# jerry102102102/RL_brain_trainer

Hardware: AMD Instinct MI355X
Metric: env-steps/sec (whole node), Stage-5 Approach->Finisher PPO loops (rollout + update); value = the Approach loop, finisher.value = the Finisher loop (higher is better)
Workload: dtype f32

## Files before the change

### rl_brain_trainer_amd/csrc/kp1_mlp.hip

```cpp
#include <hip/hip_runtime.h>
#include <hip/hip_ext.h>

#include <cmath>
#include <cstddef>
#include <cstdlib>
#include <cstring>
#include <vector>

#include "../../include/kp1_ppo.h"
#include "kp1_device.hpp"
#include "kp1_host.hpp"

using kp1::fail;
using namespace kp1;

typedef float f32x16 __attribute__((ext_vector_type(16)));
typedef float f32x4 __attribute__((ext_vector_type(4)));

namespace {

constexpr int ACT = KP1_MLP_ACT, HEADS = 8;
constexpr float LOG_SQRT_2PI = 0.9189385332046727f;

enum { EPI_BIAS_TANH = 0, EPI_DTANH = 1 };
// ... 1177 lines not shown
  if (g.reps > 1) {
    if (g.N != 128) return fail(KP1_ERR_UNSUPPORTED, "population gemm_nt is instantiated for N = 128");
    if (g.K == 64) return launch_nt_inst<128, EPI, 64, true>(g, stream);
    if (g.K == 128) return launch_nt_inst<128, EPI, 128, true>(g, stream);
    return fail(KP1_ERR_UNSUPPORTED, "population gemm_nt is instantiated for K in {64, 128}");
  }
  const int row_tiles = (g.M + 63) / 64;
  const bool wide = (g.N % 256 == 0) && row_tiles * 2 >= 200;
  if (g.K == 64) return wide ? launch_nt_inst<256, EPI, 64>(g, stream) : launch_nt_inst<128, EPI, 64>(g, stream);
  if (g.K == 128) return wide ? launch_nt_inst<256, EPI, 128>(g, stream) : launch_nt_inst<128, EPI, 128>(g, stream);
  if (g.K == 256) return wide ? launch_nt_inst<256, EPI, 256>(g, stream) : launch_nt_inst<128, EPI, 256>(g, stream);
  return fail(KP1_ERR_UNSUPPORTED, "gemm_nt is instantiated for K in {64, 128, 256}");
}

int launch_tn(kp1_mlp* m, GemmTN t, int n_o_tiles, int slab_cols, float* slab, int* n_chunks_out, hipStream_t stream);

int launch_fused(const FusedArgs& fa_in, hipStream_t stream) {
  FusedArgs fa = fa_in;
  static const int stagger_us = [] { const char* e = std::getenv("KP1_FU_STAGGER_US"); return e ? std::atoi(e) : 11; }();
  static const int n_cus = [] {
    int dev = 0, n = 0;
    if (hipGetDevice(&dev) != hipSuccess || hipDeviceGetAttribute(&n, hipDeviceAttributeMultiprocessorCount, dev) != hipSuccess) n = 256;
    return n;
  }();
  const dim3 grid((fa.n + FU_BM - 1) / FU_BM, 1, 2);
  fa.n_cus = n_cus;
  fa.stagger_ticks = (int)(grid.x * grid.z) > n_cus ? stagger_us * 100 : 0;
  const size_t bytes = sizeof(float) * FU_LDS_FLOATS;
  if (fa.sp_h1 != nullptr) {
    if (fa.inp == 64) {
      HIP_TRY(hipFuncSetAttribute((const void*)mlp_tile_kernel<true, 2, 0, true>, hipFuncAttributeMaxDynamicSharedMemorySize, (int)bytes));
      KP1_LAUNCH((mlp_tile_kernel<true, 2, 0, true>), grid, dim3(FU_NTH), bytes, stream, fa);
    } else {
      HIP_TRY(hipFuncSetAttribute((const void*)mlp_tile_kernel<true, 4, 0, true>, hipFuncAttributeMaxDynamicSharedMemorySize, (int)bytes));
      KP1_LAUNCH((mlp_tile_kernel<true, 4, 0, true>), grid, dim3(FU_NTH), bytes, stream, fa);
    }
    return KP1_OK;
  }
  if (fa.inp == 64) {
    HIP_TRY(hipFuncSetAttribute((const void*)mlp_tile_kernel<true, 2>, hipFuncAttributeMaxDynamicSharedMemorySize, (int)bytes));
    KP1_LAUNCH((mlp_tile_kernel<true, 2>), grid, dim3(FU_NTH), bytes, stream, fa);
  } else {
    HIP_TRY(hipFuncSetAttribute((const void*)mlp_tile_kernel<true, 4>, hipFuncAttributeMaxDynamicSharedMemorySize, (int)bytes));
    KP1_LAUNCH((mlp_tile_kernel<true, 4>), grid, dim3(FU_NTH), bytes, stream, fa);
  }
  return KP1_OK;
}

int launch_fused_infer_env(const FusedArgs& fa, int env_mode, hipStream_t stream) {
  const size_t bytes = sizeof(float) * FU_LDS_FLOATS;
  const dim3 grid((fa.n + FU_BM - 1) / FU_BM, 1, fa.value ? 2 : 1);
  if (env_mode == KP1_MODE_DOCK) {
    HIP_TRY(hipFuncSetAttribute((const void*)mlp_tile_kernel<false, 2, 2>, hipFuncAttributeMaxDynamicSharedMemorySize, (int)bytes));
    hipLaunchKernelGGL((mlp_tile_kernel<false, 2, 2>), grid, dim3(FU_NTH), bytes, stream, fa);
  } else {
    HIP_TRY(hipFuncSetAttribute((const void*)mlp_tile_kernel<false, 2, 1>, hipFuncAttributeMaxDynamicSharedMemorySize, (int)bytes));
    hipLaunchKernelGGL((mlp_tile_kernel<false, 2, 1>), grid, dim3(FU_NTH), bytes, stream, fa);
  }
  return KP1_OK;
}

int launch_fused_infer(const FusedArgs& fa, hipStream_t stream) {
  const size_t bytes = sizeof(float) * FU_LDS_FLOATS;
  const bool want_pi = fa.mean || fa.action || fa.clipped || fa.log_prob;
  if (!want_pi && !fa.value) return KP1_OK;
  FusedArgs f = fa;
  const bool both = want_pi && fa.value;
  if (!both) f.net_base = want_pi ? 0 : 1;
  const dim3 grid((fa.n + FU_BM - 1) / FU_BM, 1, both ? 2 : 1);
  if (fa.inp == 64) {
    HIP_TRY(hipFuncSetAttribute((const void*)mlp_tile_kernel<false, 2>, hipFuncAttributeMaxDynamicSharedMemorySize, (int)bytes));
    hipLaunchKernelGGL((mlp_tile_kernel<false, 2>), grid, dim3(FU_NTH), bytes, stream, f);
  } else {
    HIP_TRY(hipFuncSetAttribute((const void*)mlp_tile_kernel<false, 4>, hipFuncAttributeMaxDynamicSharedMemorySize, (int)bytes));
    hipLaunchKernelGGL((mlp_tile_kernel<false, 4>), grid, dim3(FU_NTH), bytes, stream, f);
  }
  return KP1_OK;
}

int launch_tn_frag(const TnFragArgs& t, hipStream_t stream) {
  if (t.n_chunks2 > 64 || t.n_chunks1 > 64) return fail(KP1_ERR_INVALID, "too many batch chunks for the partial-gradient slabs");
  const size_t bytes = sizeof(float) * TN_SPLIT_LDS_FLOATS;
  HIP_TRY(hipFuncSetAttribute((const void*)gemm_tn_split_kernel, hipFuncAttributeMaxDynamicSharedMemorySize, (int)bytes));
  KP1_LAUNCH(gemm_tn_split_kernel, dim3(32 * t.n_chunks2 + 16 * t.n_chunks1), dim3(256), bytes, stream, t);
  return KP1_OK;
}

int launch_forward_layers(kp1_mlp* m, const float* obs, int obs_stride, const int64_t* idx, int n, hipStream_t stream) {
  const int Hp = m->Hp, IN = m->L.IN, INP = m->L.INP;
  const int64_t act_stride = (int64_t)m->max_batch * Hp;
  GemmNT g{};
  g.reps = m->K;
  g.r_A = idx ? 0u : (unsigned)(n * obs_stride); g.r_gather = (unsigned)n;
  g.r_W = (unsigned)(2 * Hp * INP); g.r_bias = (unsigned)(2 * Hp); g.r_C = (unsigned)(2 * act_stride);
  g.A = obs; g.lda = obs_stride; g.strideA = 0; g.gather = idx;
  g.W = m->k.w1p; g.strideW = (int64_t)Hp * INP;
  g.bias = m->k.b1; g.strideBias = Hp;
  g.C = m->h1; g.ldc = Hp; g.strideC = act_stride;
  g.aux = nullptr; g.strideAux = 0; g.colsum = nullptr; g.strideColsum = 0;
  g.M = n; g.N = Hp; g.K = INP; g.Kreal = obs_stride >= INP ? INP : IN;
  int rc = launch_nt<EPI_BIAS_TANH>(g, stream);
  if (rc != KP1_OK) return rc;
  g.A = m->h1; g.lda = Hp; g.strideA = act_stride; g.gather = nullptr;
  g.r_A = (unsigned)(2 * act_stride); g.r_W = (unsigned)(2 * Hp * Hp);
  g.W = m->k.w2; g.strideW = (int64_t)Hp * Hp;
  g.bias = m->k.b2;
  g.C = m->h2;
  g.K = Hp; g.Kreal = Hp;
  rc = launch_nt<EPI_BIAS_TANH>(g, stream);
  if (rc != KP1_OK) return rc;
  HIP_TRY(kp1::launch_status());
  return KP1_OK;
}

}

namespace {
int launch_tn(kp1_mlp* m, GemmTN t, int n_o_tiles, int slab_cols, float* slab, int* n_chunks_out, hipStream_t stream) {
  const int Hp = m->Hp;
  const int n_chunks = (t.B + t.chunk - 1) / t.chunk;
  if (n_chunks > 64) return fail(KP1_ERR_INVALID, "too many batch chunks for the partial-gradient slab");
  t.slab = slab;
  t.slab_ld = slab_cols;
  t.slab_net_stride = (int64_t)Hp * slab_cols;
  t.slab_chunk_stride = 2 * t.slab_net_stride;
  const dim3 grid(n_chunks, n_o_tiles * t.n_i_tiles, 2 * m->K);
  if (m->K > 1) {
    t.reps = m->K;
    t.r_D = (unsigned)(2 * (int64_t)m->max_batch * Hp);
    t.r_X = t.gatherX ? 0u : t.r_D;
    t.r_gather = (unsigned)t.B;
    t.r_slab = (unsigned)(64 * t.slab_chunk_stride);
    if (t.gatherX) {
      HIP_TRY(hipFuncSetAttribute((const void*)gemm_tn_kernel<true, true>, hipFuncAttributeMaxDynamicSharedMemorySize, (int)TN_LDS_BYTES));
      hipLaunchKernelGGL((gemm_tn_kernel<true, true>), grid, dim3(256), TN_LDS_BYTES, stream, t);
    } else {
      HIP_TRY(hipFuncSetAttribute((const void*)gemm_tn_kernel<false, true>, hipFuncAttributeMaxDynamicSharedMemorySize, (int)TN_LDS_BYTES));
      hipLaunchKernelGGL((gemm_tn_kernel<false, true>), grid, dim3(256), TN_LDS_BYTES, stream, t);
    }
  } else if (t.gatherX) {
    HIP_TRY(hipFuncSetAttribute((const void*)gemm_tn_kernel<true>, hipFuncAttributeMaxDynamicSharedMemorySize, (int)TN_LDS_BYTES));
    hipLaunchKernelGGL(gemm_tn_kernel<true>, grid, dim3(256), TN_LDS_BYTES, stream, t);
  } else {
    HIP_TRY(hipFuncSetAttribute((const void*)gemm_tn_kernel<false>, hipFuncAttributeMaxDynamicSharedMemorySize, (int)TN_LDS_BYTES));
    hipLaunchKernelGGL(gemm_tn_kernel<false>, grid, dim3(256), TN_LDS_BYTES, stream, t);
  }
  if (n_chunks_out) *n_chunks_out = n_chunks;
  return KP1_OK;
}
}

extern "C" {

int64_t kp1_mlp_num_params(int32_t hidden) { return hidden > 0 ? make_layout(hidden).total : 0; }
int64_t kp1_mlp_num_params_ex(int32_t hidden, int32_t obs_dim) { return hidden > 0 && obs_dim > 0 && obs_dim <= 128 ? make_layout(hidden, obs_dim).total : 0; }

int kp1_mlp_create(int32_t device, int32_t hidden, int32_t max_batch, kp1_mlp** out) { return kp1_mlp_create_ex(device, hidden, KP1_MLP_IN, max_batch, out); }

namespace {
int mlp_create(int32_t device, int32_t hidden, int32_t obs_dim, int32_t max_batch, int32_t replicas, kp1_mlp** out);
}

int kp1_mlp_create_ex(int32_t device, int32_t hidden, int32_t obs_dim, int32_t max_batch, kp1_mlp** out) {
  return mlp_create(device, hidden, obs_dim, max_batch, 1, out);
}

int kp1_mlp_create_population(int32_t device, int32_t hidden, int32_t obs_dim, int32_t max_batch, int32_t replicas, kp1_mlp** out) {
// ... 271 lines not shown
  }
  const int hpart_stride = 10 * Hp + 32;
  if (fused) {
    FusedArgs fa{};
    fa.obs = obs; fa.obs_stride = obs_stride; fa.Kreal = obs_stride >= INP ? INP : IN; fa.inp = INP; fa.idx = idx; fa.n = n;
    fa.k = m->k;
    fa.actions = actions; fa.old_logp = old_log_prob; fa.adv = advantages; fa.ret = returns;
    fa.adv_partials = m->partials; fa.n_adv_partials = N_PARTIALS; fa.adv_stats = adv_stats_dev; fa.adv_mean = adv_mean; fa.adv_inv_std = adv_inv_std;
    fa.adv_mode = adv_mode;
    fa.clip_range = clip_range; fa.vf_coef = vf_coef; fa.inv_count = inv_count;
    fa.h1 = m->h1; fa.dz2 = m->dz2; fa.dz1 = m->dz1; fa.act_stride = act_stride; fa.xf = m->xf;
    fa.bslab = m->bslab; fa.hpart = m->hpart; fa.hpart_stride = hpart_stride;
    if (m->bf16x3) {
      fa.sp_h1 = m->sp_h1; fa.sp_dz2 = m->sp_dz2; fa.sp_dz1 = m->sp_dz1; fa.sp_xf = m->sp_xf;
      fa.sp_plane = (int64_t)2 * m->max_batch * Hp; fa.sp_plane_x = (int64_t)m->max_batch * INP;
    }
    {
      ProfScope ps(m, KP1_MLP_PROFILE_TILE, stream);
      rc = launch_fused(fa, stream);
    }
    if (rc != KP1_OK) return rc;
  } else {
    rc = launch_forward_layers(m, obs, obs_stride, idx, n, stream);
    if (rc != KP1_OK) return rc;
    HeadArgs a{};
    a.h2 = m->h2; a.strideH = act_stride; a.Hp = Hp; a.n = n; a.H = H;
    a.w3 = m->k.w3; a.b3 = m->k.b3; a.log_std = m->k.log_std;
    a.idx = idx; a.actions = actions; a.old_logp = old_log_prob; a.adv = advantages; a.ret = returns;
    a.adv_partials = m->partials; a.n_adv_partials = N_PARTIALS; a.adv_stats = adv_stats_dev; a.adv_mean = adv_mean; a.adv_inv_std = adv_inv_std;
    a.adv_mode = adv_mode;
    a.clip_range = clip_range; a.ent_coef = ent_coef; a.vf_coef = vf_coef; a.inv_count = inv_count;
    a.dz2 = m->dz2;
    a.hpart = m->hpart; a.hpart_stride = hpart_stride;
    a.r_act = (unsigned)(2 * act_stride); a.r_hpart = (unsigned)hpart_rep; a.r_partials = (unsigned)PARTIALS_STRIDE;
    a.hparams = pop && m->hparams_on ? m->hparams_dev : nullptr;
    {
      const dim3 hgrid((n + HEAD_ROWS - 1) / HEAD_ROWS, m->K);
      const size_t hbytes = sizeof(float) * (HEADS * Hp + HEAD_ROWS * 8 + 84 + 2 * HEAD_ROWS * (Hp + 4));
      if (pop) {
        HIP_TRY(hipFuncSetAttribute((const void*)head_train_kernel<128, true>, hipFuncAttributeMaxDynamicSharedMemorySize, (int)hbytes));
        hipLaunchKernelGGL((head_train_kernel<128, true>), hgrid, dim3(256), hbytes, stream, a);
      } else if (Hp == 256) {
        HIP_TRY(hipFuncSetAttribute((const void*)head_train_kernel<256>, hipFuncAttributeMaxDynamicSharedMemorySize, (int)hbytes));
        hipLaunchKernelGGL(head_train_kernel<256>, hgrid, dim3(256), hbytes, stream, a);
      } else {
        HIP_TRY(hipFuncSetAttribute((const void*)head_train_kernel<128>, hipFuncAttributeMaxDynamicSharedMemorySize, (int)hbytes));
        hipLaunchKernelGGL(head_train_kernel<128>, hgrid, dim3(256), hbytes, stream, a);
      }
    }
    GemmNT g{};
    g.A = m->dz2; g.lda = Hp; g.strideA = act_stride; g.gather = nullptr;
    g.W = m->k.w2t; g.strideW = (int64_t)Hp * Hp;
    g.bias = nullptr; g.strideBias = 0;
    g.C = m->dz1; g.ldc = Hp; g.strideC = act_stride;
    g.aux = m->h1; g.strideAux = act_stride;
    g.colsum = m->bslab; g.strideColsum = Hp;
    g.M = n; g.N = Hp; g.K = Hp; g.Kreal = Hp;
    g.reps = m->K;
    g.r_A = g.r_C = g.r_aux = (unsigned)(2 * act_stride); g.r_W = (unsigned)(2 * Hp * Hp);
    g.r_colsum = (unsigned)((m->max_batch / 32) * 2 * Hp);
    rc = launch_nt<EPI_DTANH>(g, stream);
    if (rc != KP1_OK) return rc;
  }

  int s2_n = 0, s1_n = 0;
  if (fused) {
    TnFragArgs t{};
    t.inp = INP;
    t.dz2 = m->dz2; t.h1 = m->h1; t.dz1 = m->dz1; t.act_stride = act_stride; t.xf = m->xf;
    t.slab2 = m->slab; t.s2_net = (int64_t)Hp * Hp; t.s2_chunk = 2 * t.s2_net;
    t.slab1 = m->slab1; t.s1_net = (int64_t)Hp * INP; t.s1_chunk = 2 * t.s1_net;
    t.groups = (n + FU_BM - 1) / FU_BM * (FU_BM / 8);
    auto up8 = [](int v) { return (v + 7) / 8 * 8; };
    t.cg2 = up8((t.groups + TN_SPLIT2 - 1) / TN_SPLIT2);
    t.cg1 = up8((t.groups + TN_SPLIT1 - 1) / TN_SPLIT1);
    t.n_chunks2 = (t.groups + t.cg2 - 1) / t.cg2;
    t.n_chunks1 = (t.groups + t.cg1 - 1) / t.cg1;
    if (m->bf16x3) {
      TnBf16Args b{};
      b.dz2 = m->sp_dz2; b.h1 = m->sp_h1; b.dz1 = m->sp_dz1; b.plane = (int64_t)2 * m->max_batch * Hp; b.net = (int64_t)m->max_batch * Hp;
      b.xf = m->sp_xf; b.plane_x = (int64_t)m->max_batch * INP; b.inp = INP;
      b.slab2 = t.slab2; b.s2_net = t.s2_net; b.s2_chunk = t.s2_chunk; b.slab1 = t.slab1; b.s1_net = t.s1_net; b.s1_chunk = t.s1_chunk;
      b.frags = t.groups / 2; b.cf2 = t.cg2 / 2; b.cf1 = t.cg1 / 2; b.n_chunks2 = t.n_chunks2; b.n_chunks1 = t.n_chunks1;
      const size_t bytes = sizeof(float) * TN_SPLIT_LDS_FLOATS;
      HIP_TRY(hipFuncSetAttribute((const void*)gemm_tn_bf16x3_kernel, hipFuncAttributeMaxDynamicSharedMemorySize, (int)bytes));
      ProfScope ps(m, KP1_MLP_PROFILE_WGRAD, stream);
      KP1_LAUNCH(gemm_tn_bf16x3_kernel, dim3(32 * b.n_chunks2 + 16 * b.n_chunks1), dim3(256), bytes, stream, b);
    } else {
      ProfScope ps(m, KP1_MLP_PROFILE_WGRAD, stream);
      rc = launch_tn_frag(t, stream);
    }
    if (rc != KP1_OK) return rc;
    s2_n = t.n_chunks2;
    s1_n = t.n_chunks1;
  } else {
    GemmTN t{};
    t.B = n;
    t.chunk = tn_chunk_rows(n, (Hp / 128) * (Hp / 128) * 2);
    t.D = m->dz2; t.ldd = Hp; t.strideD = act_stride;
    t.X = m->h1; t.ldx = Hp; t.strideX = act_stride; t.gatherX = nullptr;
    t.Nload = Hp; t.n_i_tiles = Hp / 128;
    rc = launch_tn(m, t, Hp / 128, Hp, m->slab, &s2_n, stream);
    if (rc != KP1_OK) return rc;
    t.D = m->dz1;
    t.X = obs; t.ldx = obs_stride; t.strideX = 0; t.gatherX = idx;
    t.Nload = obs_stride >= INP ? INP : IN; t.n_i_tiles = 1;
    t.chunk = tn_chunk_rows(n, (Hp / 128) * 2);
    rc = launch_tn(m, t, Hp / 128, INP, m->slab1, &s1_n, stream);
    if (rc != KP1_OK) return rc;
  }
  FinalizeArgs f{};
  f.L = L;
  f.slab2 = m->slab; f.s2_ld = Hp; f.s2_net = (int64_t)Hp * Hp; f.s2_chunk = 2 * f.s2_net; f.s2_n = s2_n;
  f.slab1 = m->slab1; f.s1_ld = INP; f.s1_net = (int64_t)Hp * INP; f.s1_chunk = 2 * f.s1_net; f.s1_n = s1_n;
  f.bslab = m->bslab; f.b_net = Hp; f.b_tile = 2 * Hp; f.b_n = fused ? (n + FU_BM - 1) / FU_BM * (FU_BM / 32) : nt_row_tiles(n, Hp);
  f.hpart = m->hpart; f.h_stride = 10 * Hp + 32; f.h_n = (n + HEAD_ROWS - 1) / HEAD_ROWS;
  f.ent_coef = ent_coef; f.inv_count = inv_count; f.log_std = m->k.log_std;
  f.grad = grad_out; f.stats = stats_out; f.sumsq = m->partials + 2 * N_PARTIALS;
  f.step_counter = m->step_dev;
  f.r_slab2 = (unsigned)(64 * f.s2_chunk); f.r_slab1 = (unsigned)(64 * f.s1_chunk); f.r_bslab = (unsigned)((m->max_batch / 32) * 2 * Hp);
  f.r_hpart = (unsigned)hpart_rep; f.r_sumsq = (unsigned)PARTIALS_STRIDE;
  f.hparams = pop && m->hparams_on ? m->hparams_dev : nullptr;
  const int n_main = (int)((finalize_vec_items(L) + 255) / 256);
  m->n_finalize_blocks = n_main + (int)((finalize_wide_count(L) + 3 + 31) / 32);
  if (m->n_finalize_blocks > 2048) return fail(KP1_ERR_INVALID, "parameter vector too large for the sum-of-squares partial buffer");
  {
    ProfScope ps(m, KP1_MLP_PROFILE_FINALIZE, stream);
    if (pop)
      KP1_LAUNCH(grad_finalize_kernel<true>, dim3(m->n_finalize_blocks, m->K), dim3(256), 0, stream, f, n_main);
    else
      KP1_LAUNCH(grad_finalize_kernel<false>, dim3(m->n_finalize_blocks), dim3(256), 0, stream, f, n_main);
  }
  HIP_TRY(kp1::launch_status());
  return KP1_OK;
}

int kp1_mlp_profile_read(kp1_mlp* m, float* out_us, int32_t* out_launches) {
  if (!m || !out_us || !out_launches) return fail(KP1_ERR_INVALID, "NULL argument to kp1_mlp_profile_read");
  int rc = mlp_check_device(m);
  if (rc != KP1_OK) return rc;
  for (int k = 0; k < KP1_MLP_PROFILE_SLOTS; ++k) {
    double total_ms = 0.0;
    for (int i = 0; i < m->prof_used[k]; ++i) {
      HIP_TRY(hipEventSynchronize(m->prof[k][i].b));
      float ms = 0.f;
      HIP_TRY(hipEventElapsedTime(&ms, m->prof[k][i].a, m->prof[k][i].b));
      total_ms += ms;
    }
    out_launches[k] = m->prof_used[k];
    out_us[k] = m->prof_used[k] > 0 ? (float)(total_ms * 1e3 / m->prof_used[k]) : 0.f;
    m->prof_used[k] = 0;
  }
  return KP1_OK;
}

int kp1_mlp_time_kernels(kp1_mlp* m, const float* obs, int32_t obs_stride, int32_t n, int32_t iters, float* out_ms, double* out_flops,
                         void* stream_) {
  if (!m || !obs || !out_ms || !out_flops || iters <= 0) return fail(KP1_ERR_INVALID, "bad argument to kp1_mlp_time_kernels");
  if (m->K > 1) return fail(KP1_ERR_UNSUPPORTED, "kp1_mlp_time_kernels is not available on population handles");
  if (n <= 0 || n > m->max_batch) return fail(KP1_ERR_INVALID, "n exceeds the workspace max_batch");
  int rc = mlp_check_device(m);
  if (rc != KP1_OK) return rc;
  hipStream_t stream = (hipStream_t)stream_;
  const int Hp = m->Hp, IN = m->L.IN, INP = m->L.INP;
  const int64_t act_stride = (int64_t)m->max_batch * Hp;
  hipEvent_t e0, e1;
  HIP_TRY(hipEventCreate(&e0));
// ... 78 lines not shown
  }
  (void)hipEventDestroy(e0);
  (void)hipEventDestroy(e1);
  return KP1_OK;
}

__global__ void __launch_bounds__(FU_NTH, 2) placement_probe_kernel(unsigned int* __restrict__ where, unsigned int* __restrict__ arrived, unsigned int total) {
  extern __shared__ float lds[];
  if (threadIdx.x == 0) {
    const unsigned int hw = __builtin_amdgcn_s_getreg((31 << 11) | 4);
    const unsigned int xcc = __builtin_amdgcn_s_getreg((3 << 11) | 20);
    const unsigned int linear = blockIdx.x + gridDim.x * blockIdx.z;
    where[linear] = (xcc << 16) | (((hw >> 13) & 7u) << 8) | (((hw >> 12) & 1u) << 4) | ((hw >> 8) & 15u);
    lds[0] = 0.f;
    __hip_atomic_fetch_add(arrived, 1u, __ATOMIC_RELAXED, __HIP_MEMORY_SCOPE_AGENT);
    const unsigned long long t0 = wall_clock64();
    while (__hip_atomic_load(arrived, __ATOMIC_RELAXED, __HIP_MEMORY_SCOPE_AGENT) < total && wall_clock64() - t0 < 200000ull) __builtin_amdgcn_s_sleep(8);
  }
  __syncthreads();
}

int kp1_mlp_placement_check(int32_t device, int32_t n_rows, int32_t* out, void* stream_) {
  if (!out || n_rows <= 0) return fail(KP1_ERR_INVALID, "bad argument to kp1_mlp_placement_check");
  HIP_TRY(hipSetDevice(device));
  hipStream_t stream = (hipStream_t)stream_;
  int n_cus = 0;
  HIP_TRY(hipDeviceGetAttribute(&n_cus, hipDeviceAttributeMultiprocessorCount, device));
  const dim3 grid((n_rows + FU_BM - 1) / FU_BM, 1, 2);
  const unsigned int total = grid.x * grid.z;
  if ((int)total > 2 * n_cus) return fail(KP1_ERR_UNSUPPORTED, "placement probe: the grid must be resident at once");
  unsigned int* dev = nullptr;
  HIP_TRY(hipMalloc(&dev, sizeof(unsigned int) * (total + 1)));
  HIP_TRY(hipMemsetAsync(dev, 0, sizeof(unsigned int) * (total + 1), stream));
  const size_t bytes = sizeof(float) * FU_LDS_FLOATS;
  HIP_TRY(hipFuncSetAttribute((const void*)placement_probe_kernel, hipFuncAttributeMaxDynamicSharedMemorySize, (int)bytes));
  hipLaunchKernelGGL(placement_probe_kernel, grid, dim3(FU_NTH), bytes, stream, dev, dev + total, total);
  std::vector<unsigned int> host(total + 1);
  hipError_t e = hipMemcpyAsync(host.data(), dev, sizeof(unsigned int) * (total + 1), hipMemcpyDeviceToHost, stream);
  if (e == hipSuccess) e = hipStreamSynchronize(stream);
  (void)hipFree(dev);
  HIP_TRY(e);
  int pairs = 0, same = 0, rr = 0;
  std::vector<unsigned int> seen;
  for (unsigned int k = 0; k < total; ++k) {
    if ((host[k] >> 16) == (host[k & 7u] >> 16)) ++rr;
    if (k + (unsigned)n_cus < total) {
      ++pairs;
      if (host[k] == host[k + n_cus]) ++same;
    }
    bool fresh = true;
    for (unsigned int v : seen) fresh = fresh && v != host[k];
    if (fresh) seen.push_back(host[k]);
  }
  int xcds = 0;
  for (unsigned int a = 0; a < 8 && a < total; ++a) {
    bool fresh = true;
    for (unsigned int b = 0; b < a; ++b) fresh = fresh && (host[a] >> 16) != (host[b] >> 16);
    xcds += fresh ? 1 : 0;
  }
  out[0] = (int)total; out[1] = pairs; out[2] = same; out[3] = rr; out[4] = n_cus; out[5] = (int)seen.size(); out[6] = (int)host[total]; out[7] = xcds;
  return KP1_OK;
}

#ifdef KP1_CLK_TRACE
int kp1_debug_clk_trace(unsigned long long* out) {
  HIP_TRY(hipDeviceSynchronize());
  HIP_TRY(hipMemcpyFromSymbol(out, HIP_SYMBOL(kp1_clk_buf), sizeof(unsigned long long) * 2 * 1024 * 4));
  return KP1_OK;
}
#endif

#ifdef KP1_NT_TRACE
int kp1_debug_nt_trace(unsigned long long* out, int clear) {
  HIP_TRY(hipDeviceSynchronize());
  if (out) HIP_TRY(hipMemcpyFromSymbol(out, HIP_SYMBOL(kp1_nt_trace_buf), sizeof(unsigned long long) * KP1_TRACE_SLOTS * KP1_TRACE_WGS));
  if (clear) {
    std::vector<unsigned long long> z(KP1_TRACE_SLOTS * KP1_TRACE_WGS, 0ull);
    HIP_TRY(hipMemcpyToSymbol(HIP_SYMBOL(kp1_nt_trace_buf), z.data(), sizeof(unsigned long long) * z.size()));
  }
  return KP1_OK;
}
#endif

int kp1_mlp_adam_step(kp1_mlp* m, float* params, float* grad, float* exp_avg, float* exp_avg_sq, float lr, float eps, float max_grad_norm,
                      int32_t step, int32_t zero_grad, void* stream_) {
  if (!m || !params || !grad || !exp_avg || !exp_avg_sq) return fail(KP1_ERR_INVALID, "bad argument to kp1_mlp_adam_step");
  int rc = mlp_check_device(m);
  if (rc != KP1_OK) return rc;
  hipStream_t stream = (hipStream_t)stream_;
  const int64_t n = m->L.total;
  const bool fused_norm = (zero_grad & 2) && m->n_finalize_blocks > 0;
  const double* norm_partials = fused_norm ? m->partials + 2 * N_PARTIALS : m->partials + N_PARTIALS;
  const int n_norm_partials = fused_norm ? m->n_finalize_blocks : N_PARTIALS;
  ProfScope ps(m, KP1_MLP_PROFILE_ADAM, stream);
  const bool pop = m->K > 1;
  if (!fused_norm) {
    if (pop)
      hipLaunchKernelGGL(sumsq_partials_kernel<true>, dim3(N_PARTIALS, m->K), dim3(256), 0, stream, grad, n, m->partials + N_PARTIALS, (unsigned)PARTIALS_STRIDE);
    else
      hipLaunchKernelGGL(sumsq_partials_kernel<false>, dim3(N_PARTIALS), dim3(256), 0, stream, grad, n, m->partials + N_PARTIALS, 0u);
  }
  zero_grad = 0;
  const int host_step = step > 0 ? step : 1;
  const float bc1 = 1.f - std::pow(0.9f, (float)host_step);
  const float bc2 = 1.f - std::pow(0.999f, (float)host_step);
  Packed kfmt = m->k;
  const bool frag_only = m->fused && m->Hp == FU_HP;
  kfmt.formats = frag_only ? PACK_FRAG : (PACK_SLAB | PACK_FRAG);
  m->last_params = params;
  if (frag_only) m->slab_stale = true;
  const int* step_arg = step > 0 ? (const int*)nullptr : (const int*)m->step_dev;
  if (pop)
    KP1_LAUNCH(adam_kernel<true>, dim3((unsigned)((n + ADAM_BLOCK - 1) / ADAM_BLOCK), m->K), dim3(ADAM_BLOCK), 0, stream, params, grad, exp_avg, exp_avg_sq, n,
               norm_partials, n_norm_partials, lr, eps, max_grad_norm, bc1, std::sqrt(bc2), m->L, kfmt, zero_grad, step_arg, host_step,
               (const int*)m->step_dev + 1, (unsigned)PARTIALS_STRIDE, m->hparams_on ? (const float*)m->hparams_dev : (const float*)nullptr);
  else
    KP1_LAUNCH(adam_kernel<false>, dim3((unsigned)((n + ADAM_BLOCK - 1) / ADAM_BLOCK)), dim3(ADAM_BLOCK), 0, stream, params, grad, exp_avg, exp_avg_sq, n, norm_partials,
               n_norm_partials, lr, eps, max_grad_norm, bc1, std::sqrt(bc2), m->L, kfmt, zero_grad, step_arg, host_step, (const int*)m->step_dev + 1, 0u,
               (const float*)nullptr);
  HIP_TRY(kp1::launch_status());
  return KP1_OK;
}

}
```

### rl_brain_trainer_amd/csrc/kp1_mlp_fused.inc

```

struct TnFragArgs {
  const float* dz2; const float* h1; const float* dz1; int64_t act_stride;
  const float* xf; int inp;
  float* slab2; int64_t s2_net, s2_chunk;
  float* slab1; int64_t s1_net, s1_chunk;
  int groups, cg2, n_chunks2, cg1, n_chunks1;
};

template <int RA, int CB>
__device__ __forceinline__ void tn_split_tile(const float* __restrict__ Af, int a_ncb, const float* __restrict__ Bf, int b_ncb, int g_begin, int g_end,
                                              float* __restrict__ out, int out_ld, float* lds) {
  constexpr int SG = 4;
  const int tid = threadIdx.x, lane = tid & 63, wave = __builtin_amdgcn_readfirstlane(tid >> 6);
  const int per = (max(g_end - g_begin, 0) + 3) >> 2;
  const int gb = min(g_begin + wave * per, g_end), ge = min(gb + per, g_end);
  const int64_t a_gs = (int64_t)a_ncb * 256, b_gs = (int64_t)b_ncb * 256;
  f32x4 ra[2][SG][RA], rb[2][SG][CB];
  f32x16 acc[RA][CB];
#pragma unroll
  for (int r = 0; r < RA; ++r)
#pragma unroll
    for (int c = 0; c < CB; ++c)
#pragma unroll
      for (int e = 0; e < 16; ++e) acc[r][c][e] = 0.f;
  KP1_TR(12)
  KP1_TR_HW(11)
  if (gb < ge) {
    const int g_last = ge - 1;
#define KP1_TNS_LOAD(set, g0)                                                                           \
  _Pragma("unroll") for (int u = 0; u < SG; ++u) {                                                      \
    const int gg_ = min((g0) + u, g_last);                                                              \
    _Pragma("unroll") for (int r = 0; r < RA; ++r) ra[set][u][r] = load16_sc1(Af, lane * 4 + gg_ * a_gs + r * 256); \
    _Pragma("unroll") for (int c = 0; c < CB; ++c) rb[set][u][c] = load16_sc1(Bf, lane * 4 + gg_ * b_gs + c * 256); \
  }
#define KP1_TNS_MFMA(set, g0)                                                                           \
  _Pragma("unroll") for (int u = 0; u < SG; ++u) {                                                      \
    const float keep_ = (g0) + u < ge ? 1.f : 0.f;                                                      \
    _Pragma("unroll") for (int i = 0; i < 4; ++i)                                                       \
      _Pragma("unroll") for (int r = 0; r < RA; ++r)                                                    \
        _Pragma("unroll") for (int c = 0; c < CB; ++c)                                                  \
          acc[r][c] = __builtin_amdgcn_mfma_f32_32x32x2f32(ra[set][u][r][i] * keep_, rb[set][u][c][i], acc[r][c], 0, 0, 0); \
  }
    KP1_TNS_LOAD(0, gb)
    for (int g = gb; g < ge; g += 2 * SG) {
      KP1_TNS_LOAD(1, g + SG)
      __builtin_amdgcn_sched_barrier(0);
      KP1_TNS_MFMA(0, g)
      __builtin_amdgcn_sched_barrier(0);
      KP1_TNS_LOAD(0, g + 2 * SG)
      __builtin_amdgcn_sched_barrier(0);
      KP1_TNS_MFMA(1, g + SG)
      __builtin_amdgcn_sched_barrier(0);
    }
#undef KP1_TNS_LOAD
#undef KP1_TNS_MFMA
  }
  KP1_TR(13)
  constexpr int TO = 32 * RA, TI = 32 * CB, LDP = TI + 8, Q = TI / 4;
  float* mine = lds + wave * (TO * LDP);
#pragma unroll
  for (int r = 0; r < RA; ++r)
#pragma unroll
    for (int c = 0; c < CB; ++c)
#pragma unroll
      for (int e = 0; e < 16; ++e) {
        const int o = r * 32 + (e & 3) + 8 * (e >> 2) + 4 * (lane >> 5);
        mine[o * LDP + c * 32 + (lane & 31)] = acc[r][c][e];
      }
  __syncthreads();
  KP1_TR(14)
#pragma unroll
  for (int j = 0; j < TO * Q / 256; ++j) {
    const int f = tid + 256 * j, o = f / Q, q = f % Q;
    const float* p0 = lds + o * LDP + 4 * q;
    const f32x4 v = ((*reinterpret_cast<const f32x4*>(p0) + *reinterpret_cast<const f32x4*>(p0 + TO * LDP)) +
                     *reinterpret_cast<const f32x4*>(p0 + 2 * TO * LDP)) + *reinterpret_cast<const f32x4*>(p0 + 3 * TO * LDP);
    store16_sc1(out, (int64_t)o * out_ld + 4 * q, v);
  }
  KP1_TR(15)
}
constexpr int TN_SPLIT_LDS_FLOATS = 4 * 64 * (64 + 8);

__global__ void __launch_bounds__(256, 2) gemm_tn_split_kernel(const TnFragArgs a) {
  extern __shared__ float lds[];
  KP1_CLK(1, 0)
  const int n2 = 32 * a.n_chunks2;
  if ((int)blockIdx.x < n2) {
    const int chunk = blockIdx.x % a.n_chunks2, tile = blockIdx.x / a.n_chunks2;
    const int net = tile >> 4, ot = (tile >> 2) & 3, it = tile & 3;
    const int g0 = chunk * a.cg2, g1 = min(g0 + a.cg2, a.groups);
    float* out = a.slab2 + chunk * a.s2_chunk + net * a.s2_net + (int64_t)(ot * 64) * FU_HP + it * 64;
    tn_split_tile<2, 2>(a.dz2 + net * a.act_stride + (ot * 2) * 256, 8, a.h1 + net * a.act_stride + (it * 2) * 256, 8, g0, g1, out, FU_HP, lds);
  } else {
    const int id = blockIdx.x - n2;
    const int chunk = id % a.n_chunks1, tile = id / a.n_chunks1;
    const int net = tile >> 3, ot = tile & 7;
    const int g0 = chunk * a.cg1, g1 = min(g0 + a.cg1, a.groups);
    const int inp = a.inp;
    float* out = a.slab1 + chunk * a.s1_chunk + net * a.s1_net + (int64_t)(ot * 32) * inp;
    if (inp == 64)
      tn_split_tile<1, 2>(a.dz1 + net * a.act_stride + ot * 256, 8, a.xf, 2, g0, g1, out, 64, lds);
    else
      tn_split_tile<1, 3>(a.dz1 + net * a.act_stride + ot * 256, 8, a.xf, 4, g0, g1, out, 128, lds);
  }
  KP1_CLK(1, 1)
}

struct TnBf16Args {
  const unsigned short* dz2; const unsigned short* h1; const unsigned short* dz1; int64_t plane, net;
  const unsigned short* xf; int64_t plane_x; int inp;
  float* slab2; int64_t s2_net, s2_chunk;
  float* slab1; int64_t s1_net, s1_chunk;
  int frags, cf2, n_chunks2, cf1, n_chunks1;
};

__device__ __forceinline__ bf16x8 tnb_load(const unsigned short* __restrict__ base, int64_t off) {
  const __amdgpu_buffer_rsrc_t r = __builtin_amdgcn_make_buffer_rsrc(const_cast<unsigned short*>(base), 0, 0x7fffffff, 0x00020000);
  return __builtin_bit_cast(bf16x8, __builtin_amdgcn_raw_buffer_load_b128(r, (int)(off * 2), 0, AUX_SC1));
}

template <int RA, int CB>
__device__ __forceinline__ void tn_bf16_tile(const unsigned short* __restrict__ Af, int64_t a_plane, int a_ncb, const unsigned short* __restrict__ Bf, int64_t b_plane,
                                             int b_ncb, int f_begin, int f_end, float* __restrict__ out, int out_ld, float* lds) {
  const int tid = threadIdx.x, lane = tid & 63, wave = __builtin_amdgcn_readfirstlane(tid >> 6);
  const int per = (max(f_end - f_begin, 0) + 3) >> 2;
  const int fb = min(f_begin + wave * per, f_end), fe = min(fb + per, f_end);
  const int64_t a_fs = (int64_t)a_ncb * 512, b_fs = (int64_t)b_ncb * 512;
  bf16x8 ra[2][3][RA], rb[2][3][CB];
  f32x16 acc[RA][CB];
#pragma unroll
  for (int r = 0; r < RA; ++r)
#pragma unroll
    for (int c = 0; c < CB; ++c)
#pragma unroll
      for (int e = 0; e < 16; ++e) acc[r][c][e] = 0.f;
  if (fb < fe) {
    const int f_last = fe - 1;
#define KP1_TNB_LOAD(set, f0)                                                                           \
  {                                                                                                     \
    const int ff_ = min((f0), f_last);                                                                  \
    _Pragma("unroll") for (int pl = 0; pl < 3; ++pl) {                                                  \
      _Pragma("unroll") for (int r = 0; r < RA; ++r) ra[set][pl][r] = tnb_load(Af, lane * 8 + pl * a_plane + ff_ * a_fs + r * 512); \
      _Pragma("unroll") for (int c = 0; c < CB; ++c) rb[set][pl][c] = tnb_load(Bf, lane * 8 + pl * b_plane + ff_ * b_fs + c * 512); \
    }                                                                                                   \
  }
#define KP1_TNB_MFMA(set)                                                                               \
  _Pragma("unroll") for (int r = 0; r < RA; ++r)                                                        \
    _Pragma("unroll") for (int c = 0; c < CB; ++c) {                                                    \
      acc[r][c] = __builtin_amdgcn_mfma_f32_32x32x16_bf16(ra[set][2][r], rb[set][0][c], acc[r][c], 0, 0, 0);   \
      acc[r][c] = __builtin_amdgcn_mfma_f32_32x32x16_bf16(ra[set][0][r], rb[set][2][c], acc[r][c], 0, 0, 0);   \
      acc[r][c] = __builtin_amdgcn_mfma_f32_32x32x16_bf16(ra[set][1][r], rb[set][1][c], acc[r][c], 0, 0, 0);   \
      acc[r][c] = __builtin_amdgcn_mfma_f32_32x32x16_bf16(ra[set][0][r], rb[set][1][c], acc[r][c], 0, 0, 0);   \
      acc[r][c] = __builtin_amdgcn_mfma_f32_32x32x16_bf16(ra[set][1][r], rb[set][0][c], acc[r][c], 0, 0, 0);   \
      acc[r][c] = __builtin_amdgcn_mfma_f32_32x32x16_bf16(ra[set][0][r], rb[set][0][c], acc[r][c], 0, 0, 0);   \
    }
    KP1_TNB_LOAD(0, fb)
    int f = fb;
    for (; f + 1 < fe; f += 2) {
      KP1_TNB_LOAD(1, f + 1)
      __builtin_amdgcn_sched_barrier(0);
      KP1_TNB_MFMA(0)
      __builtin_amdgcn_sched_barrier(0);
      KP1_TNB_LOAD(0, f + 2)
      __builtin_amdgcn_sched_barrier(0);
      KP1_TNB_MFMA(1)
      __builtin_amdgcn_sched_barrier(0);
    }
    if (f < fe) { KP1_TNB_MFMA(0) }
#undef KP1_TNB_LOAD
#undef KP1_TNB_MFMA
  }
  constexpr int TO = 32 * RA, TI = 32 * CB, LDP = TI + 8, Q = TI / 4;
  float* mine = lds + wave * (TO * LDP);
#pragma unroll
  for (int r = 0; r < RA; ++r)
#pragma unroll
    for (int c = 0; c < CB; ++c)
#pragma unroll
      for (int e = 0; e < 16; ++e) {
        const int o = r * 32 + (e & 3) + 8 * (e >> 2) + 4 * (lane >> 5);
        mine[o * LDP + c * 32 + (lane & 31)] = acc[r][c][e];
      }
  __syncthreads();
#pragma unroll
  for (int j = 0; j < TO * Q / 256; ++j) {
    const int fq = tid + 256 * j, o = fq / Q, q = fq % Q;
    const float* p0 = lds + o * LDP + 4 * q;
    const f32x4 v = ((*reinterpret_cast<const f32x4*>(p0) + *reinterpret_cast<const f32x4*>(p0 + TO * LDP)) +
                     *reinterpret_cast<const f32x4*>(p0 + 2 * TO * LDP)) + *reinterpret_cast<const f32x4*>(p0 + 3 * TO * LDP);
    store16_sc1(out, (int64_t)o * out_ld + 4 * q, v);
  }
}

__global__ void __launch_bounds__(256, 2) gemm_tn_bf16x3_kernel(const TnBf16Args a) {
  extern __shared__ float lds[];
  const int n2 = 32 * a.n_chunks2;
  if ((int)blockIdx.x < n2) {
    const int chunk = blockIdx.x % a.n_chunks2, tile = blockIdx.x / a.n_chunks2;
    const int net = tile >> 4, ot = (tile >> 2) & 3, it = tile & 3;
    const int f0 = chunk * a.cf2, f1 = min(f0 + a.cf2, a.frags);
    float* out = a.slab2 + chunk * a.s2_chunk + net * a.s2_net + (int64_t)(ot * 64) * FU_HP + it * 64;
    tn_bf16_tile<2, 2>(a.dz2 + net * a.net + (ot * 2) * 512, a.plane, 8, a.h1 + net * a.net + (it * 2) * 512, a.plane, 8, f0, f1, out, FU_HP, lds);
  } else {
    const int id = blockIdx.x - n2;
    const int chunk = id % a.n_chunks1, tile = id / a.n_chunks1;
    const int net = tile >> 3, ot = tile & 7;
    const int f0 = chunk * a.cf1, f1 = min(f0 + a.cf1, a.frags);
    const int inp = a.inp;
    float* out = a.slab1 + chunk * a.s1_chunk + net * a.s1_net + (int64_t)(ot * 32) * inp;
    if (inp == 64)
      tn_bf16_tile<1, 2>(a.dz1 + net * a.net + ot * 512, a.plane, 8, a.xf, a.plane_x, 2, f0, f1, out, 64, lds);
    else
      tn_bf16_tile<1, 3>(a.dz1 + net * a.net + ot * 512, a.plane, 8, a.xf, a.plane_x, 4, f0, f1, out, 128, lds);
  }
}
```

Measured before the change: 11.42 million.

## Split TN weight-gradient tiles into smaller blocks for more parallelism and occupancy

The fp32 split-K weight-gradient kernel now uses 32x64 (and 32x32) output tiles instead of 64x64/32x96, doubling the dW2 block count and splitting the dW1 block for INP=128 into two pieces, with the mapping factored into a shared host/device helper. The LDS footprint is halved, so the launch bound is raised to 3 blocks per CU. The intent is to fill more CUs and hide latency on small batches, at the cost of re-loading operand fragments across more blocks. The bf16x3 path keeps its old LDS size through a separate constant, and debug entry points for the block map and finalize partials are added.

```diff
diff --git a/rl_brain_trainer_amd/csrc/kp1_mlp.hip b/rl_brain_trainer_amd/csrc/kp1_mlp.hip
--- a/rl_brain_trainer_amd/csrc/kp1_mlp.hip
+++ b/rl_brain_trainer_amd/csrc/kp1_mlp.hip
@@ -1283,7 +1283,7 @@
   if (t.n_chunks2 > 64 || t.n_chunks1 > 64) return fail(KP1_ERR_INVALID, "too many batch chunks for the partial-gradient slabs");
   const size_t bytes = sizeof(float) * TN_SPLIT_LDS_FLOATS;
   HIP_TRY(hipFuncSetAttribute((const void*)gemm_tn_split_kernel, hipFuncAttributeMaxDynamicSharedMemorySize, (int)bytes));
-  KP1_LAUNCH(gemm_tn_split_kernel, dim3(32 * t.n_chunks2 + 16 * t.n_chunks1), dim3(256), bytes, stream, t);
+  KP1_LAUNCH(gemm_tn_split_kernel, dim3(tn_grid_blocks(t.n_chunks2, t.n_chunks1, t.inp)), dim3(256), bytes, stream, t);
   return KP1_OK;
 }
 
@@ -1721,7 +1721,7 @@
       b.xf = m->sp_xf; b.plane_x = (int64_t)m->max_batch * INP; b.inp = INP;
       b.slab2 = t.slab2; b.s2_net = t.s2_net; b.s2_chunk = t.s2_chunk; b.slab1 = t.slab1; b.s1_net = t.s1_net; b.s1_chunk = t.s1_chunk;
       b.frags = t.groups / 2; b.cf2 = t.cg2 / 2; b.cf1 = t.cg1 / 2; b.n_chunks2 = t.n_chunks2; b.n_chunks1 = t.n_chunks1;
-      const size_t bytes = sizeof(float) * TN_SPLIT_LDS_FLOATS;
+      const size_t bytes = sizeof(float) * TN_BF16_LDS_FLOATS;
       HIP_TRY(hipFuncSetAttribute((const void*)gemm_tn_bf16x3_kernel, hipFuncAttributeMaxDynamicSharedMemorySize, (int)bytes));
       ProfScope ps(m, KP1_MLP_PROFILE_WGRAD, stream);
       KP1_LAUNCH(gemm_tn_bf16x3_kernel, dim3(32 * b.n_chunks2 + 16 * b.n_chunks1), dim3(256), bytes, stream, b);
@@ -1966,6 +1966,23 @@
 }
 #endif
 
+int kp1_debug_finalize_sumsq(kp1_mlp* m, double* out, int32_t cap, int32_t* n) {
+  if (!m || !out || !n || cap < m->n_finalize_blocks) return fail(KP1_ERR_INVALID, "bad argument to kp1_debug_finalize_sumsq");
+  HIP_TRY(hipDeviceSynchronize());
+  HIP_TRY(hipMemcpy(out, m->partials + 2 * N_PARTIALS, sizeof(double) * m->n_finalize_blocks, hipMemcpyDeviceToHost));
+  *n = m->n_finalize_blocks;
+  return KP1_OK;
+}
+
+int kp1_debug_tn_block_map(int32_t inp, int32_t n_chunks2, int32_t n_chunks1, int32_t block, int32_t* out) {
+  if (!out || (inp != 64 && inp != 128) || n_chunks2 < 1 || n_chunks1 < 1) return fail(KP1_ERR_INVALID, "bad argument to kp1_debug_tn_block_map");
+  out[0] = tn_grid_blocks(n_chunks2, n_chunks1, inp);
+  if (block < 0 || block >= out[0]) return KP1_OK;
+  const TnBlock k = tn_block_map(block, n_chunks2, n_chunks1, inp);
+  out[1] = k.dw1; out[2] = k.net; out[3] = k.a_cb0; out[4] = k.b_cb0; out[5] = k.b_ncb; out[6] = k.chunk;
+  return KP1_OK;
+}
+
 int kp1_mlp_adam_step(kp1_mlp* m, float* params, float* grad, float* exp_avg, float* exp_avg_sq, float lr, float eps, float max_grad_norm,
                       int32_t step, int32_t zero_grad, void* stream_) {
   if (!m || !params || !grad || !exp_avg || !exp_avg_sq) return fail(KP1_ERR_INVALID, "bad argument to kp1_mlp_adam_step");
diff --git a/rl_brain_trainer_amd/csrc/kp1_mlp_fused.inc b/rl_brain_trainer_amd/csrc/kp1_mlp_fused.inc
--- a/rl_brain_trainer_amd/csrc/kp1_mlp_fused.inc
+++ b/rl_brain_trainer_amd/csrc/kp1_mlp_fused.inc
@@ -79,30 +79,46 @@
   }
   KP1_TR(15)
 }
-constexpr int TN_SPLIT_LDS_FLOATS = 4 * 64 * (64 + 8);
-
-__global__ void __launch_bounds__(256, 2) gemm_tn_split_kernel(const TnFragArgs a) {
+constexpr int TN_SPLIT_LDS_FLOATS = 4 * 32 * (64 + 8);
+
+struct TnBlock { int dw1, net, a_cb0, b_cb0, b_ncb, chunk; };
+__host__ __device__ inline int tn_dw1_pieces(int inp) { return inp == 64 ? 1 : 2; }
+__host__ __device__ inline int tn_grid_blocks(int n_chunks2, int n_chunks1, int inp) { return 64 * n_chunks2 + 16 * tn_dw1_pieces(inp) * n_chunks1; }
+__host__ __device__ inline TnBlock tn_block_map(int block, int n_chunks2, int n_chunks1, int inp) {
+  TnBlock k;
+  const int n2 = 64 * n_chunks2;
+  if (block < n2) {
+    const int tile = block / n_chunks2, half = tile & 1, it = (tile >> 1) & 3, ot = (tile >> 3) & 3;
+    k.dw1 = 0; k.chunk = block % n_chunks2; k.net = tile >> 5;
+    k.a_cb0 = 2 * ot + half; k.b_cb0 = 2 * it; k.b_ncb = 2;
+  } else {
+    const int id = block - n2, pieces = tn_dw1_pieces(inp), tile = id / n_chunks1, piece = tile % pieces, t = tile / pieces;
+    k.dw1 = 1; k.chunk = id % n_chunks1; k.net = t >> 3;
+    k.a_cb0 = t & 7; k.b_cb0 = 2 * piece; k.b_ncb = 2 - piece;
+  }
+  return k;
+}
+
+__global__ void __launch_bounds__(256, 3) gemm_tn_split_kernel(const TnFragArgs a) {
   extern __shared__ float lds[];
   KP1_CLK(1, 0)
-  const int n2 = 32 * a.n_chunks2;
-  if ((int)blockIdx.x < n2) {
-    const int chunk = blockIdx.x % a.n_chunks2, tile = blockIdx.x / a.n_chunks2;
-    const int net = tile >> 4, ot = (tile >> 2) & 3, it = tile & 3;
-    const int g0 = chunk * a.cg2, g1 = min(g0 + a.cg2, a.groups);
-    float* out = a.slab2 + chunk * a.s2_chunk + net * a.s2_net + (int64_t)(ot * 64) * FU_HP + it * 64;
-    tn_split_tile<2, 2>(a.dz2 + net * a.act_stride + (ot * 2) * 256, 8, a.h1 + net * a.act_stride + (it * 2) * 256, 8, g0, g1, out, FU_HP, lds);
+  const TnBlock k = tn_block_map(blockIdx.x, a.n_chunks2, a.n_chunks1, a.inp);
+  const float *A, *B;
+  float* out;
+  int b_blocks, cg;
+  if (!k.dw1) {
+    A = a.dz2 + k.net * a.act_stride; B = a.h1 + k.net * a.act_stride; b_blocks = 8; cg = a.cg2;
+    out = a.slab2 + k.chunk * a.s2_chunk + k.net * a.s2_net;
   } else {
-    const int id = blockIdx.x - n2;
-    const int chunk = id % a.n_chunks1, tile = id / a.n_chunks1;
-    const int net = tile >> 3, ot = tile & 7;
-    const int g0 = chunk * a.cg1, g1 = min(g0 + a.cg1, a.groups);
-    const int inp = a.inp;
-    float* out = a.slab1 + chunk * a.s1_chunk + net * a.s1_net + (int64_t)(ot * 32) * inp;
-    if (inp == 64)
-      tn_split_tile<1, 2>(a.dz1 + net * a.act_stride + ot * 256, 8, a.xf, 2, g0, g1, out, 64, lds);
-    else
-      tn_split_tile<1, 3>(a.dz1 + net * a.act_stride + ot * 256, 8, a.xf, 4, g0, g1, out, 128, lds);
-  }
+    A = a.dz1 + k.net * a.act_stride; B = a.xf; b_blocks = a.inp >> 5; cg = a.cg1;
+    out = a.slab1 + k.chunk * a.s1_chunk + k.net * a.s1_net;
+  }
+  const int ld = 32 * b_blocks, g0 = k.chunk * cg, g1 = min(g0 + cg, a.groups);
+  A += k.a_cb0 * 256; B += k.b_cb0 * 256; out += (int64_t)(32 * k.a_cb0) * ld + 32 * k.b_cb0;
+  if (k.b_ncb == 2)
+    tn_split_tile<1, 2>(A, 8, B, b_blocks, g0, g1, out, ld, lds);
+  else
+    tn_split_tile<1, 1>(A, 8, B, b_blocks, g0, g1, out, ld, lds);
   KP1_CLK(1, 1)
 }
 
@@ -191,6 +207,8 @@
     store16_sc1(out, (int64_t)o * out_ld + 4 * q, v);
   }
 }
+
+constexpr int TN_BF16_LDS_FLOATS = 4 * 64 * (64 + 8);
 
 __global__ void __launch_bounds__(256, 2) gemm_tn_bf16x3_kernel(const TnBf16Args a) {
   extern __shared__ float lds[];
```

After: 11.58 million, median of 6. 1.01x the previous value.
